# santurini/vsrlab

Measured on AMD Instinct MI355X. Metric: LR frames/sec fwd+bwd, BasicVSR 4x 540p 7-frame clip, 1->8 MI355X, higher is better.
Workload: dtype bf16; 1 GPU; BasicVSR(mid=64,res_blocks=30,x4) fwd+Charbonnier+bwd+clip+Adam, 540x960->2160x3840, 7-frame clip, 2 clips per GPU (BASELINE configs[1]); clips_per_gpu=2, frames=7, res_blocks=30, parallelism=single GPU, arena=full, train_flow=False, trunk_chains=True

## Files before the change

include/vsrlab_hip.h:

```cpp
#ifndef VSRLAB_HIP_H
#define VSRLAB_HIP_H
#include <stddef.h>
#ifdef __cplusplus
extern "C" {
#endif

#define VSR_DT_F32 0
#define VSR_DT_BF16 1

#define VSR_STATUS_OK 0
#define VSR_STATUS_BADARG (-1)
#define VSR_STATUS_UNSUPPORTED (-2)
#define VSR_STATUS_HIP (-3)
#define VSR_STATUS_WORKSPACE (-4)

int vsr_abi_version(void);
const char* vsr_status_string(int status);

typedef struct VsrBasicVSRDesc {
    int n, t, h, w;
    int mid_channels;
    int res_blocks;
    int upscale;
    int dtype;
// ... 66 lines not shown

int vsr_planar_to_pm(int dtype, const float* in, void* out_pm, int N, int Cin, int H, int W, int C,
                     void* stream);
int vsr_pm_to_planar(int dtype, const void* in_pm, float* out, int N, int Cout, int H, int W, int C,
                     void* stream);

int vsr_conv3x3_c64_fwd(int dtype, const void* x_pm, const float* w, const float* b, void* wpack,
                        void* y_pm, const void* res_pm, int act, int N, int H, int W, void* stream);

size_t vsr_conv3x3_c64_chain_sync_bytes(int nlayers, int N, int H, int W);
int vsr_conv3x3_c64_chain_fwd(const void* images, const void* wpack, const float* bias, int nlayers, int N, int H, int W,
                              void* sync, void* stream);
int vsr_conv3x3_c64_dgrad(int dtype, const void* dy_pm, const float* w, void* wpack, void* dx_pm,
                          const void* res_pm, const void* aux_pm, int mask_mode, int N, int H,
                          int W, void* stream);
int vsr_conv_layer_fwd(int dtype, int ks, const void* x_pm, int cin_pm, const float* lr_planar, const float* w,
                       const float* b, int cin_real, int cout_real, void* wpack, void* y_pm, int cd, float* y_planar,
                       int act, float slope, int pixel_shuffle, int N, int H, int W, void* stream);
size_t vsr_conv_layer_bwd_scratch_bytes(int dtype, int N, int H, int W, int pixel_shuffle);
int vsr_conv_layer_bwd(int dtype, int ks, const void* x_pm, int cin_pm, const float* lr_planar, const float* w, int cin_real,
                       int cout_real, const void* y_pm, const float* y_planar, const void* dy_pm, const float* dy_planar, int cd,
                       int act, float slope, int pixel_shuffle, void* dx_pm, float* dlr_planar, float* gw, float* gb,
                       void* scratch, size_t scratch_bytes, int N, int H, int W, void* stream);
size_t vsr_conv3x3_c64_wgrad_slab_floats(void);
int vsr_conv3x3_c64_wgrad(int dtype, const void* x_pm, const void* dy_pm, float* gw, float* gb,
                          float* slab, int N, int H, int W, void* stream);

size_t vsr_charbonnier_scratch_floats(void);
int vsr_charbonnier_fwd_bwd(const float* sr, const float* hr, float* dsr, float* loss, float* scratch, long long numel,
                            float eps, void* stream);
// ... 47 lines not shown
```

vsrlab_amd/_lib.py:

```python
import ctypes
import os
from ctypes import c_char_p, c_float, c_int, c_longlong, c_size_t, c_void_p

_HERE = os.path.dirname(os.path.abspath(__file__))
LIB_PATH = os.environ.get("VSRLAB_AMD_LIB") or os.path.join(_HERE, "lib", "libvsrlab_hip.so")

DT_F32 = 0
DT_BF16 = 1


class BasicVSRDesc(ctypes.Structure):
    _fields_ = [("n", c_int), ("t", c_int), ("h", c_int), ("w", c_int), ("mid_channels", c_int),
                ("res_blocks", c_int), ("upscale", c_int), ("dtype", c_int), ("arena_mode", c_int)]


class DiscDesc(ctypes.Structure):
    _fields_ = [("n", c_int), ("h", c_int), ("w", c_int), ("mid_ch", c_int), ("dtype", c_int)]


class AttnDesc(ctypes.Structure):
    _fields_ = [(k, c_int) for k in ("B", "N", "heads", "head_dim", "q0", "k0", "o0", "Nq", "Nk", "Cout", "c_off", "nW", "Nm")] + \
               [("scale", c_float), ("dtype", c_int), ("mask_packed", c_int), ("mask_value", c_float)]


# ... 19 lines not shown
    "vsr_cleaner_narrow_workspace_bytes": (c_size_t, [c_int, c_int, c_int, c_int, c_int, c_int, c_int, c_int]),
    "vsr_cleaner_forward": (c_int, [c_int, c_int, c_int, c_int, c_int, c_int, c_int, _P, c_int, _P, _P, _P, c_size_t, c_int, _P]),
    "vsr_cleaner_backward": (c_int, [c_int, c_int, c_int, c_int, c_int, c_int, c_int, _P, c_int, _P, _P, _P, _P, c_size_t, _P]),
    "vsr_flow_warp_fwd": (c_int, [c_int, _P, _P, _P, c_int, c_int, c_int, c_int, _P]),
    "vsr_flow_warp_bwd": (c_int, [c_int, _P, _P, _P, c_int, c_int, c_int, c_int, _P]),
    "vsr_flow_warp_bwd_flow": (c_int, [c_int, _P, _P, _P, _P, c_int, c_int, c_int, c_int, _P]),
    "vsr_flow_warp_fwd_ex": (c_int, [c_int, _P, _P, _P, c_int, c_int, c_int, c_int, c_int, _P]),
    "vsr_flow_warp_bwd_ex": (c_int, [c_int, _P, _P, _P, c_int, c_int, c_int, c_int, c_int, _P]),
    "vsr_flow_warp_bwd_flow_ex": (c_int, [c_int, _P, _P, _P, _P, c_int, c_int, c_int, c_int, c_int, _P]),
    "vsr_planar_to_pm": (c_int, [c_int, _P, _P, c_int, c_int, c_int, c_int, c_int, _P]),
    "vsr_pm_to_planar": (c_int, [c_int, _P, _P, c_int, c_int, c_int, c_int, c_int, _P]),
    "vsr_conv3x3_c64_fwd": (c_int, [c_int, _P, _P, _P, _P, _P, _P, c_int, c_int, c_int, c_int, _P]),
    "vsr_conv3x3_c64_chain_sync_bytes": (c_size_t, [c_int, c_int, c_int, c_int]),
    "vsr_conv3x3_c64_chain_fwd": (c_int, [_P, _P, _P, c_int, c_int, c_int, c_int, _P, _P]),
    "vsr_conv3x3_c64_dgrad": (c_int, [c_int, _P, _P, _P, _P, _P, _P, c_int, c_int, c_int, c_int, _P]),
    "vsr_conv_layer_fwd": (c_int, [c_int, c_int, _P, c_int, _P, _P, _P, c_int, c_int, _P, _P, c_int, _P, c_int, c_float, c_int, c_int, c_int, c_int, _P]),
    "vsr_conv_layer_bwd_scratch_bytes": (c_size_t, [c_int, c_int, c_int, c_int, c_int]),
    "vsr_conv_layer_bwd": (c_int, [c_int, c_int, _P, c_int, _P, _P, c_int, c_int, _P, _P, _P, _P, c_int, c_int, c_float, c_int, _P, _P, _P, _P,
                                   _P, c_size_t, c_int, c_int, c_int, _P]),
    "vsr_conv3x3_c64_wgrad_slab_floats": (c_size_t, []),
    "vsr_conv3x3_c64_wgrad": (c_int, [c_int, _P, _P, _P, _P, _P, c_int, c_int, c_int, _P]),
    "vsr_charbonnier_scratch_floats": (c_size_t, []),
    "vsr_charbonnier_fwd_bwd": (c_int, [_P, _P, _P, _P, _P, c_longlong, c_float, _P]),
    "vsr_optim_scratch_floats": (c_size_t, []),
    "vsr_adam_clip_step": (c_int, [_P, _P, _P, _P, c_longlong, c_float, c_float, c_float, c_float, c_float, c_int, c_float,
                                   c_float, _P, _P, _P]),
    "vsr_grad_norm": (c_int, [_P, c_longlong, c_float, _P, _P, _P]),
    "vsr_resize_bilinear": (c_int, [_P, _P, c_longlong, c_int, c_int, c_int, c_int, _P]),
    "vsr_disc_workspace_bytes": (c_size_t, [ctypes.POINTER(DiscDesc), c_int]),
    "vsr_disc_forward": (c_int, [ctypes.POINTER(DiscDesc), _P, c_int, _P, _P, _P, c_size_t, c_int, _P]),
# ... 36 lines not shown
```

vsrlab_amd/csrc/common.h:

```cpp
#pragma once
#include <hip/hip_runtime.h>
#include <stdint.h>

#define VSR_OK 0
#define VSR_ERR_BADARG (-1)
#define VSR_ERR_UNSUPPORTED (-2)
#define VSR_ERR_HIP (-3)
#define VSR_ERR_WORKSPACE (-4)

#define VSR_F32 0
#define VSR_BF16 1

typedef __bf16 bf16_t;
typedef __attribute__((ext_vector_type(8))) __bf16 bf16x8_t;
typedef __attribute__((ext_vector_type(4))) __bf16 bf16x4_t;
typedef __attribute__((ext_vector_type(4))) short s16x4_t;
typedef __attribute__((ext_vector_type(16))) float f32x16_t;
typedef __attribute__((ext_vector_type(4))) float f32x4_t;

#define VSR_MAX_SRC 4
#define VSR_MAX_Z 4

enum { ACT_NONE = 0, ACT_RELU = 1, ACT_LEAKY = 2 };
enum { MASK_NONE = 0, MASK_RELU = 1, MASK_LEAKY = 2, MASK_RELU_BITS = 3, MASK_LEAKY_BITS = 4 };
// ... 18 lines not shown
    int cout_real;
    int act;
    const void* res[VSR_MAX_Z];
    const void* aux[VSR_MAX_Z];
    int mask_mode;
    const float* pres;
    const float* base_lr;
    long long base_nstride;
    int base_h, base_w, base_scale;
    void* sign_out[VSR_MAX_Z];
    const void* sign_bits[VSR_MAX_Z];
    float leaky_slope;
    int planar_c;
    int unshuffle;
    long long unshuffle_plane;
};
static inline __host__ __device__ float vsr_slope(float s) { return s != 0.f ? s : 0.1f; }

#define VSR_WG_MAXSEG 8
struct WgradArgs {
    const void* x[VSR_WG_MAXSEG];
    const void* dy[VSR_WG_MAXSEG];
    long long x_nstride, dy_nstride;
    int nseg;
    int N, H, W;
    int x_step, x_oy, x_ox, Hx, Wx;
    int dy_step, dy_oy, dy_ox, Hy, Wy;
    float* slab;
    int tap_begin;
    int x_ctotal, x_coff;
// ... 83 lines not shown
```

vsrlab_amd/csrc/conv3x3_persist.hip:

```cpp
#include "common.h"
#include <type_traits>

namespace {

constexpr int PTW = 32, PTH = 8, PNT = 512;
constexpr int PTWH = PTW + 2, PTHH = PTH + 2, PNPIX = PTHH * PTWH;
constexpr int W_BYTES = 9 * 64 * 64 * 2;
constexpr int IN_BYTES = PNPIX * 128;
constexpr int BIAS_OFF = W_BYTES + 2 * IN_BYTES;
constexpr int P_LDS = BIAS_OFF + 256;
constexpr int IN_CHUNKS = PNPIX * 8;
constexpr int NPIECE_T = (IN_CHUNKS + 63) / 64;
constexpr int NPIECE_W = (NPIECE_T + 3) / 4;

__device__ uint4 g_conv_zero_chunk[2];

template <int ACT> __device__ __forceinline__ float p_act(float v, float slope) {
    if (ACT == ACT_RELU) return v > 0.f ? v : 0.f;
    if (ACT == ACT_LEAKY) return v > 0.f ? v : slope * v;
    return v;
}

#ifdef VSR_STAMPS
__device__ unsigned long long g_stamps[256 * 8 * 8];
// ... 55 lines not shown
__device__ __forceinline__ unsigned pk_max_i16(unsigned a, unsigned b) { unsigned r; asm("v_pk_max_i16 %0, %1, %2" : "=v"(r) : "v"(a), "v"(b)); return r; }
__device__ __forceinline__ unsigned pk_min_u16(unsigned a, unsigned b) { unsigned r; asm("v_pk_min_u16 %0, %1, %2" : "=v"(r) : "v"(a), "v"(b)); return r; }
__device__ __forceinline__ unsigned pk_mul_lo_u16(unsigned a, unsigned b) { unsigned r; asm("v_pk_mul_lo_u16 %0, %1, %2" : "=v"(r) : "v"(a), "v"(b)); return r; }

#ifdef VSR_ABL
#define P_DMA_AUX (((VSR_ABL >> 8) & 1) ? 2 : 0)
#define P_NT_STORE ((VSR_ABL >> 9) & 1)
#else
#define P_DMA_AUX 0
#define P_NT_STORE 0
#endif
#define GLDS16(src, dst)                                                                              \
    __builtin_amdgcn_global_load_lds((const __attribute__((address_space(1))) void*)(src),            \
                                     (__attribute__((address_space(3))) void*)(dst), 16, 0, P_DMA_AUX)

template <int ACT, bool HAS_RES, int MASK>
__global__ __launch_bounds__(PNT, 1) void conv3x3_c64_persist_kernel(const ConvArgs ka) {
    extern __shared__ __attribute__((aligned(16))) char smem[];

    const int z = blockIdx.y;
    struct {
        int N, H, W, Ws, Wd, in_step, out_step, src_ox0, src_oy0, out_oxz, out_oyz, bias_zstride, unshuffle;
        long long src_nstride0, dst_nstride, w_zstride, plane;
        unsigned long long src0, wpack, resz, auxz, sign_bitsz, dstz, sign_outz, bias; float leaky_slope;
    } a = {ka.N, ka.H, ka.W, ka.Ws, ka.Wd, ka.in_step, ka.out_step, ka.src_ox[0], ka.src_oy[0], ka.out_ox[z], ka.out_oy[z], ka.bias_zstride, ka.unshuffle,
           ka.src_nstride[0], ka.dst_nstride, ka.w_zstride, ka.unshuffle_plane,
           (unsigned long long)ka.src[0], (unsigned long long)ka.wpack, (unsigned long long)ka.res[z], (unsigned long long)ka.aux[z],
           (unsigned long long)ka.sign_bits[z], (unsigned long long)ka.dst[z], (unsigned long long)ka.sign_out[z], (unsigned long long)ka.bias, ka.leaky_slope};
    asm volatile("" : "+s"(a.N), "+s"(a.H), "+s"(a.W), "+s"(a.Ws), "+s"(a.Wd), "+s"(a.in_step), "+s"(a.out_step), "+s"(a.src_ox0), "+s"(a.src_oy0),
                 "+s"(a.out_oxz), "+s"(a.out_oyz), "+s"(a.bias_zstride), "+s"(a.unshuffle), "+s"(a.src_nstride0), "+s"(a.dst_nstride), "+s"(a.w_zstride), "+s"(a.plane));
    asm volatile("" : "+s"(a.src0), "+s"(a.wpack), "+s"(a.resz), "+s"(a.auxz), "+s"(a.sign_bitsz), "+s"(a.dstz), "+s"(a.sign_outz), "+s"(a.bias), "+s"(a.leaky_slope));
#define GP(T, x) ((__attribute__((address_space(1))) T*)(x))
    const int tid = threadIdx.x, lane = tid & 63, wave = tid >> 6;
    const int role = __builtin_amdgcn_readfirstlane(wave >> 2);
    const int w4 = wave & 3;
    const int l15 = lane & 15, q = lane >> 4;
    const int pxl = (l15 >= 4 && l15 < 12) ? 2 * (l15 - 4) : (l15 < 4 ? 2 * l15 + 1 : 2 * (l15 - 8) + 1);
    char* lds_w = smem;
#ifdef VSR_STAMPS
    const unsigned long long st_begin = stamp();
    unsigned long long st_sum[8] = {0, 0, 0, 0, 0, 0, 0, 0};
#endif
    char* lds_t = smem + W_BYTES;
#ifdef VSR_ABL
    unsigned long long clk_t0 = 0, clk_r0 = 0;
// ... 22 lines not shown
        *reinterpret_cast<u32x4_t*>(lds_w + tap * 8192 + (r * 8 + (c ^ ((r >> 1) & 7))) * 16) = wv[i];                     \
    }

    if (role == 1) {
        const auto* src = GP(const char, a.src0);
        const auto* zsrc = GP(const char, g_conv_zero_chunk);
        int rel[NPIECE_W];
#pragma unroll
        for (int i = 0; i < NPIECE_W; ++i) {
            const int idx = (w4 + 4 * i) * 64 + lane;
            const int ty = idx / (8 * PTWH), rem = idx - ty * (8 * PTWH);
            const int c = rem / PTWH, tx = rem - c * PTWH;
            const int dx = (tx - 1) * a.in_step + a.src_ox0;
            rel[i] = (((((ty - 1) * a.in_step + a.src_oy0) * WSs + (dx >> 5)) * 8 + c) * 256 + (dx & 31) * 8) * 2;
        }
        auto issue = [&](const TileIter& it, int buf) {
            const int n = it.n, ty0 = it.ty * PTH, tx0 = it.tx * PTW;
            const auto* org = src + ((long long)n * a.src_nstride0 + pm_off(ty0 * a.in_step, tx0 * a.in_step, 0, a.Ws, 64)) * 2;
            char* dstb = lds_t + buf * IN_BYTES;
            if (ty0 >= 1 && ty0 + PTH < a.H && tx0 >= 1 && tx0 + PTW < a.W) {
#pragma unroll
                for (int i = 0; i < NPIECE_W; ++i) {
                    const int piece = w4 + 4 * i;
                    if (piece < NPIECE_T && piece * 64 + lane < IN_CHUNKS) GLDS16(org + rel[i], dstb + piece * 1024);
                }
            } else {
#pragma unroll
                for (int i = 0; i < NPIECE_W; ++i) {
                    const int piece = w4 + 4 * i;
                    const int idx = piece * 64 + lane;
                    const int ty = idx / (8 * PTWH), rem = idx - ty * (8 * PTWH);
                    const int tx = rem % PTWH;
                    const int vy = ty0 + ty - 1, vx = tx0 + tx - 1;
                    const auto* s = (vy >= 0 && vy < a.H && vx >= 0 && vx < a.W) ? org + rel[i] : zsrc;
                    if (piece < NPIECE_T && idx < IN_CHUNKS) GLDS16(s, dstb + piece * 1024);
                }
            }
        };
        int cur = 0;
        TileIter it;
        it.init(walk.first, walk.stride, ntx, nty);
        STAMP(q0);
        if (it.tile < walk.end) issue(it, 0);
        STAMP(q1);
        STAMP_ADD(1, st_begin, q0);
        asm volatile("s_waitcnt vmcnt(0)" ::: "memory");
        STAMP(q3);
        __syncthreads();
        STAMP_ADD(2, st_begin, q1); STAMP_ADD(4, q1, q3);
        while (it.tile < walk.end) {
            STAMP(t0);
            it.advance(walk.stride, ntx, nty);
            if (it.tile < walk.end && !ABL(3)) issue(it, cur ^ 1);
            STAMP(p1);
            asm volatile("s_waitcnt vmcnt(0)" ::: "memory");
            STAMP(p2);
            __syncthreads();
            STAMP(p3);
            STAMP_ADD(5, t0, p1); STAMP_ADD(6, p1, p2); STAMP_ADD(7, p2, p3);
            cur ^= 1;
        }
    } else {
        STAMP(m0);
        u32x4_t wv[WCH];
        W_LOAD(wv)
        unsigned a_lo[2], a_hi[2];
#pragma unroll
        for (int kk = 0; kk < 2; ++kk) {
            a_lo[kk] = (unsigned)((l15 * 8 + ((4 * kk + q) ^ ((l15 >> 1) & 7))) * 16);
            a_hi[kk] = a_lo[kk] + 6 * 8192;
        }
        const int b_lane = w4 * 2 * (PTWH * 128) + q * (PTWH * 16) + pxl * 16;
        int loff[4];
#pragma unroll
        for (int nb = 0; nb < 4; ++nb) {
            const int dx = ((nb & 1) * 16 + pxl) * a.out_step + a.out_oxz;
            loff[nb] = ((((w4 * 2 + (nb >> 1)) * a.out_step) * WSd + (dx >> 5)) * 8 + q) * 256 + (dx & 31) * 8;
            if (a.unshuffle) {
                const int row = w4 * 2 + (nb >> 1), px = (nb & 1) * 16 + pxl;
                loff[nb] = (int)(((row & 1) * 2 + (px & 1)) * a.plane) + (((row >> 1) * pm_ws(a.Wd >> 1)) * 8 + q) * 256 + (px >> 1) * 8;
            }
        }
        W_STORE(wv)
        STAMP(m1);
        STAMP_ADD(6, m0, m1);
        asm volatile("s_waitcnt vmcnt(0)" ::: "memory");
        __syncthreads();
#ifdef VSR_STAMPS
        st_sum[5] = stamp() - st_begin;
#endif
        auto* const dst_z = GP(bf16_t, a.dstz);
        const auto* const res_z = GP(const bf16_t, a.resz);
        const auto* const aux_z = GP(const bf16_t, a.auxz);
        const auto* const sbits_z = GP(const u32x2_t, a.sign_bitsz);
        auto* const sout_z = GP(u32x2_t, a.sign_outz);
        const float slope = vsr_slope(a.leaky_slope);

        f32x4_t bvec[4];
#pragma unroll
        for (int mb = 0; mb < 4; ++mb) bvec[mb] = *reinterpret_cast<const f32x4_t*>(smem + BIAS_OFF + (mb * 16 + 4 * q) * 4);
        bf16x8_t idA[2];
#pragma unroll
        for (int hb = 0; hb < 2; ++hb)
#pragma unroll
            for (int j = 0; j < 8; ++j) idA[hb][j] = (bf16_t)((q == (l15 >> 2) && j == 4 * hb + (l15 & 3)) ? 1.f : 0.f);
        constexpr bool RES_MFMA = HAS_RES && !ABL(4);

        int cur = 0;
        TileIter it;
        for (it.init(walk.first, walk.stride, ntx, nty); it.tile < walk.end; it.advance(walk.stride, ntx, nty)) {
            STAMP(t0);
            const int tile = it.tile, n = it.n, ty0 = it.ty * PTH, tx0 = it.tx * PTW;
            const long long tbase = a.unshuffle ? (long long)n * a.dst_nstride + pm_off(ty0 >> 1, tx0 >> 1, 0, a.Wd >> 1, 64)
                                                : (long long)n * a.dst_nstride + pm_off(ty0 * a.out_step + a.out_oyz, tx0 * a.out_step, 0, a.Wd, 64);
            const bool full = ty0 + PTH <= a.H && tx0 + PTW <= a.W;
            bool ok[4];
            constexpr bool BITS = MASK == MASK_RELU_BITS || MASK == MASK_LEAKY_BITS;
            constexpr bool LATE_MASK = HAS_RES && MASK != MASK_NONE && !BITS;
            u32x4_t rr[2][4], mm[2][4];
            u32x2_t sbits = {0u, 0u};
            if (BITS) sbits = sbits_z[(long long)tile * 256 + w4 * 64 + lane];
#pragma unroll
            for (int nb = 0; nb < 4; ++nb) ok[nb] = (tx0 + (nb & 1) * 16 + pxl < a.W) && (ty0 + w4 * 2 + (nb >> 1) < a.H);
#define CV_OPERANDS(OKN)                                                                                               \
            _Pragma("unroll") for (int nb = 0; nb < 4; ++nb) {                                                         \
                if (OKN) {                                                                                             \
                    _Pragma("unroll") for (int k = 0; k < 2; ++k) {                                                    \
                        const long long o = tbase + loff[nb] + k * 1024;                                               \
                        if (HAS_RES) rr[k][nb] = *GP(const u32x4_t, res_z + o);                                        \
                        if (MASK != MASK_NONE && !LATE_MASK && !BITS) mm[k][nb] = *GP(const u32x4_t, aux_z + o);       \
                    }                                                                                                  \
                }                                                                                                      \
            }
            if (HAS_RES || (MASK != MASK_NONE && !LATE_MASK && !BITS)) {
                if (full) { CV_OPERANDS(true) } else { CV_OPERANDS(ok[nb]) }
            }
#undef CV_OPERANDS
            STAMP(t1);

            f32x4_t acc[4][4];

            bf16x8_t fa[2][4], fb[2][4];
            const unsigned bb = (unsigned)(W_BYTES + cur * IN_BYTES + b_lane);
#define DSR(dst, addr, imm) asm volatile("ds_read_b128 %0, %1 offset:%2" : "=v"(dst) : "v"(addr), "i"(imm))
#define CV_LOADA(tap_, kk_, slot, mb)                                                                                  \
            if (!(ABL(2) && tap_ >= 6) && !(ABL(6) && tap_ + kk_ > 0)) DSR(fa[slot][mb], (tap_ < 6 ? a_lo[kk_] : a_hi[kk_]), (tap_ < 6 ? tap_ : tap_ - 6) * 8192 + (mb) * 2048);
#define CV_LOADB(ky_, kx_, kk_, slot, nb)                                                                              \
            if (!(ABL(0) && ky_ == 2) && !(ABL(6) && ky_ + kx_ + kk_ > 0)) DSR(fb[slot][nb], bb, (((nb) >> 1) + ky_) * (PTWH * 128) + kk_ * (4 * PTWH * 16) + (((nb) & 1) * 16 + kx_) * 16);
#define CV_LOAD(s, slot)                                                                                               \
// ... 15 lines not shown
            __builtin_amdgcn_sched_barrier(0);
#define CV_STEP(s)                                                                                                     \
            {                                                                                                          \
                if (!ABL(7)) asm volatile("s_waitcnt lgkmcnt(0)" ::: "memory");              \
                __builtin_amdgcn_sched_barrier(0);                                                                     \
                CV_ML_A(s, 0, 0, 0) CV_ML_A(s, 0, 1, 1) CV_ML_A(s, 0, 2, 2) CV_ML_A(s, 0, 3, 3)                        \
                CV_ML_B(s, 1, 0, 0) CV_ML_B(s, 1, 1, 1) CV_ML_B(s, 1, 2, 2) CV_ML_B(s, 1, 3, 3)                        \
                CV_MFMA(s, 2, 0) CV_MFMA(s, 2, 1) CV_MFMA(s, 2, 2) CV_MFMA(s, 2, 3)                                    \
                CV_MFMA(s, 3, 0) CV_MFMA(s, 3, 1) CV_MFMA(s, 3, 2) CV_MFMA(s, 3, 3)                                    \
                __builtin_amdgcn_sched_barrier(0);                                                                     \
            }
            asm volatile("s_waitcnt lgkmcnt(0)" ::: "memory");
            __builtin_amdgcn_sched_barrier(0);
            CV_LOAD(0, 0)
            CV_STEP(0) CV_STEP(1) CV_STEP(2) CV_STEP(3) CV_STEP(4) CV_STEP(5) CV_STEP(6) CV_STEP(7) CV_STEP(8)
            CV_STEP(9) CV_STEP(10) CV_STEP(11) CV_STEP(12) CV_STEP(13) CV_STEP(14) CV_STEP(15) CV_STEP(16) CV_STEP(17)
#undef CV_ML_A
#undef CV_ML_B
#undef CV_STEP
#undef CV_MFMA
#undef CV_LOAD
#undef CV_LOADB
#undef CV_LOADA
#undef DSR
            STAMP(t2);

            if (HAS_RES || MASK != MASK_NONE) __builtin_amdgcn_s_waitcnt(0x0F70);
            if constexpr (RES_MFMA) {
#pragma unroll
                for (int nb = 0; nb < 4; ++nb)
#pragma unroll
                    for (int mb = 0; mb < 4; ++mb)
                        acc[mb][nb] = __builtin_amdgcn_mfma_f32_16x16x32_bf16(idA[mb & 1], __builtin_bit_cast(bf16x8_t, rr[mb >> 1][nb]), acc[mb][nb], 0, 0, 0);
            }
            unsigned sout[2] = {0u, 0u};
            const unsigned k11 = 0x00010001u;
            auto epilogue = [&](auto FULL) {
#pragma unroll
            for (int nb = 0; nb < 4; ++nb) {
                if (decltype(FULL)::value || ok[nb]) {
                    auto* dst = dst_z + tbase + loff[nb];
#pragma unroll
                    for (int k = 0; k < 2; ++k) {
                        float v[8];
#pragma unroll
                        for (int j = 0; j < 4; ++j) { v[j] = acc[2 * k][nb][j]; v[4 + j] = acc[2 * k + 1][nb][j]; }
                        const unsigned wbits = k ? sbits.y : sbits.x;
                        unsigned ow[4];
// ... 16 lines not shown
#pragma unroll
                            for (int jj = 0; jj < 4; ++jj)
                                ow[jj] = pk_mul_lo_u16(pk_bf16(v[2 * jj], v[2 * jj + 1]), (wbits >> (4 * nb + jj)) & k11);
                        } else {
#pragma unroll
                            for (int j = 0; j < 8; ++j) v[j] = p_act<ACT>(v[j], slope);
                            if (HAS_RES && !(RES_MFMA && ACT == ACT_NONE)) {
                                const unsigned rw[4] = {rr[k][nb].x, rr[k][nb].y, rr[k][nb].z, rr[k][nb].w};
#pragma unroll
                                for (int jj = 0; jj < 4; ++jj) { v[2 * jj] += bf_lo(rw[jj]); v[2 * jj + 1] += bf_hi(rw[jj]); }
                            }
                            if (ACT != ACT_NONE && !HAS_RES && !ABL(1)) {
#pragma unroll
                                for (int j = 0; j < 8; ++j) sout[k] |= (v[j] > 0.f ? 1u : 0u) << (4 * nb + (j >> 1) + 16 * (j & 1));
                            }
                            if (BITS) {
                                const float neg = MASK == MASK_LEAKY_BITS ? slope : 0.f;
#pragma unroll
                                for (int j = 0; j < 8; ++j) v[j] *= ((wbits >> (4 * nb + (j >> 1) + 16 * (j & 1))) & 1u) ? 1.f : neg;
                            } else if (MASK != MASK_NONE) {
                                const float neg = MASK == MASK_LEAKY ? slope : 0.f;
                                u32x4_t mq = mm[k][nb];
                                if (LATE_MASK) mq = *GP(const u32x4_t, aux_z + tbase + loff[nb] + k * 1024);
                                const unsigned mw[4] = {mq.x, mq.y, mq.z, mq.w};
#pragma unroll
                                for (int jj = 0; jj < 4; ++jj) {
                                    v[2 * jj] *= (bf_lo(mw[jj]) > 0.f ? 1.f : neg);
                                    v[2 * jj + 1] *= (bf_hi(mw[jj]) > 0.f ? 1.f : neg);
                                }
                            }
#pragma unroll
                            for (int jj = 0; jj < 4; ++jj) ow[jj] = pk_bf16(v[2 * jj], v[2 * jj + 1]);
                        }
                        const u32x4_t o = {ow[0], ow[1], ow[2], ow[3]};
                        if (P_NT_STORE) __builtin_nontemporal_store(o, GP(u32x4_t, dst + k * 1024));
                        else if (!ABL(5)) *GP(u32x4_t, dst + k * 1024) = o;
                        else asm volatile("" :: "v"(o.x), "v"(o.y), "v"(o.z), "v"(o.w));
                    }
                }
            }
            };
            if (full) epilogue(std::true_type{}); else epilogue(std::false_type{});
            if (ACT != ACT_NONE && !HAS_RES && sout_z && !ABL(1)) sout_z[(long long)tile * 256 + w4 * 64 + lane] = u32x2_t{sout[0], sout[1]};
            STAMP(t3);
            __syncthreads();
            cur ^= 1;
            STAMP(t4);
            STAMP_ADD(1, t0, t1); STAMP_ADD(2, t1, t2); STAMP_ADD(3, t2, t3); STAMP_ADD(4, t3, t4);
        }
    }
// ... 27 lines not shown
        const int yy = ty0 + 2 * w4 + (nb >> 1), xx = tx0 + (nb & 1) * 16 + pxl;
        if (yy < H && xx < W) {
#pragma unroll
            for (int k = 0; k < 2; ++k) {
                const uint4 v = *reinterpret_cast<const uint4*>(x + (long long)n * pm_image_elems(H, W, 64) + pm_off(yy, xx, 4 * k + q, W, 64));
                const unsigned vw[4] = {v.x, v.y, v.z, v.w};
#pragma unroll
                for (int jj = 0; jj < 4; ++jj)
                    out[k] |= ((bf_lo(vw[jj]) > 0.f ? 1u : 0u) | (bf_hi(vw[jj]) > 0.f ? 0x10000u : 0u)) << (4 * nb + jj);
            }
        }
    }
    bits[gid] = make_uint2(out[0], out[1]);
}

template <int ACT, bool HAS_RES, int MASK>
static int launch_persist(const ConvArgs& a, int num_cus, hipStream_t st) {
    auto kern = conv3x3_c64_persist_kernel<ACT, HAS_RES, MASK>;
    static VsrDevOnce once;
    { const int rc = vsr_set_max_dynamic_lds(once, reinterpret_cast<const void*>(kern), P_LDS); if (rc != VSR_OK) return rc; }
    const int tiles = a.N * cdiv(a.W, PTW) * cdiv(a.H, PTH);
    int gx = num_cus / a.nz;
    gx &= ~7;
    if (gx < 8) gx = num_cus / a.nz;
    if (gx < 1) gx = 1;
    if (gx > tiles) gx = tiles;
    hipLaunchKernelGGL(kern, dim3(gx, a.nz), dim3(PNT), P_LDS, st, a);
    HIP_CHECK_RET(hipGetLastError());
    return VSR_OK;
}

}

// ... 33 lines not shown
    }
#define PERSIST_CASE(ACT, RES, MASK) if (a.act == ACT && res == RES && mask == MASK) return launch_persist<ACT, RES, MASK>(a, num_cus, st);
    PERSIST_CASE(ACT_RELU, false, MASK_NONE)
    PERSIST_CASE(ACT_NONE, true, MASK_NONE)
    PERSIST_CASE(ACT_LEAKY, false, MASK_NONE)
    PERSIST_CASE(ACT_NONE, false, MASK_NONE)
    PERSIST_CASE(ACT_NONE, false, MASK_RELU)
    PERSIST_CASE(ACT_NONE, false, MASK_RELU_BITS)
    PERSIST_CASE(ACT_NONE, true, MASK_LEAKY)
    PERSIST_CASE(ACT_NONE, true, MASK_LEAKY_BITS)
    PERSIST_CASE(ACT_NONE, false, MASK_LEAKY)
#undef PERSIST_CASE
    return VSR_ERR_UNSUPPORTED;
}

int vsr_launch_sign_bits_c64(const void* x_pm, void* bits, int N, int H, int W, hipStream_t st) {
    if (!x_pm || !bits || N < 1 || H < 1 || W < 1) return VSR_ERR_BADARG;
    const long long total = (long long)N * cdiv(W, PTW) * cdiv(H, PTH) * 256;
    hipLaunchKernelGGL(sign_bits_c64_kernel, dim3((unsigned)((total + 255) / 256)), dim3(256), 0, st, (const bf16_t*)x_pm, (uint2*)bits, N, H, W);
    HIP_CHECK_RET(hipGetLastError());
    return VSR_OK;
}
```

vsrlab_amd/csrc/engine.hip:

```cpp
#include <vector>
#include "kernels.h"
#include "../../include/vsrlab_hip.h"

namespace {

struct Bump {
    size_t off = 0;
    size_t take(size_t bytes) {
        size_t o = off;
        off += (bytes + 255) & ~size_t(255);
        return o;
    }
};

inline size_t esize(int dtype) { return dtype == VSR_BF16 ? 2 : 4; }

constexpr int C = 64;
constexpr int NSPY = 5;
const int SPY_CI[NSPY] = {8, 32, 64, 32, 16}, SPY_CO[NSPY] = {32, 64, 32, 16, 2};
const int SPY_CIP[NSPY] = {16, 32, 64, 32, 16}, SPY_COP[NSPY] = {32, 64, 32, 32, 32};
const int SPY_CD[NSPY] = {32, 64, 32, 16, 0};
const int SPY_DK[NSPY] = {32, 64, 32, 16, 16}, SPY_DROWS[NSPY] = {32, 32, 64, 32, 32};

struct SpyPlan {
// ... 170 lines not shown
                    G1[dir].assign((size_t)t * rb, 0); DX[dir].assign((size_t)t * (rb + 1), 0);
                    for (int i = 0; i < t; ++i) {
                        for (int k = 0; k < rb; ++k) G1[dir][(size_t)i * rb + k] = b.take(a1);
                        for (int k = 1; k <= rb; ++k) DX[dir][(size_t)i * (rb + 1) + k] = b.take(a1);
                    }
                } else {
                    G1[dir] = G1[0]; DX[dir] = DX[0];
                }
            }
            dFeatB.assign(t, 0); dFF.assign(t, 0);
            for (int i = 0; i < t; ++i) { dFeatB[i] = b.take(a1); dFF[i] = b.take(a1); }
            for (int dir = 0; dir < 2; ++dir) { S[dir] = b.take(s_elems * 8); dWp[dir] = b.take(a1); }
            far_cnt = b.take((size_t)2 * 32 * 4);
            G_C0 = b.take(a4h); G_P = b.take(a1);
            unsh = !diet && dtype == VSR_BF16 && !vsr_env().generic_conv && C == 64;
            const size_t gu1 = unsh && 4 * a2 > a4 ? 4 * a2 : a4, gu0 = unsh && 4 * a1 > a2 ? 4 * a1 : a2;
            if (ups == 2) { if (diet) { G_U1 = C0[0]; G_U0 = U1[0]; } else { G_U1 = b.take(gu1); G_U0 = b.take(gu0); } }
            else { G_U0 = diet ? C0[0] : b.take(gu0); G_U1 = G_U0; }
            hrdef = unsh;
            GU1f.assign(t, G_U1); GU0f.assign(t, G_U0); GPf.assign(t, G_P);
            if (hrdef)
                for (int i = 1; i < t; ++i) {
                    GU0f[i] = b.take(gu0);
                    GU1f[i] = ups == 2 ? b.take(gu1) : GU0f[i];
                    GPf[i] = b.take(a1);
                }
            int cp, xp, stride;
            vsr_wgrad_slab_dims(3, 64, 64, &cp, &xp, &stride);
            for (int k = 0; k < 2; ++k) slab[k] = b.take((size_t)VSR_WGRAD_NWG * stride * 4);
        }
// ... 43 lines not shown
        if (unshuffle) set_unshuffle(a, N, H, W);
        if (p.C != 64) return vsr_launch_conv(dtype, 3, 1, p.C, p.C, 0, p.CO, EPI_NHWC, a, st);
        const int rc = vsr_launch_conv(dtype, 3, 1, 64, 64, 0, 64, EPI_NHWC, a, st);
        if (rc == VSR_OK && sign_out && dtype == VSR_BF16 && vsr_env().generic_conv) return vsr_launch_sign_bits_c64(y, sign_out, N, H, W, st);
        return rc;
    }
    int conv_ps(const void* x, size_t wpack, const float* bias4, void* y, int N, int H, int W) const {
        const int C = p.C;
        ConvArgs a = base(N, H, W);
        a.src[0] = x; a.wpack = at(wpack); a.w_zstride = 9 * p.CO * C; a.bias = bias4; a.bias_zstride = C; a.nz = 4;
        a.out_step = 2; a.Hd = 2 * H; a.Wd = 2 * W; a.dst_nstride = pm_image_elems(2 * H, 2 * W, C);
        for (int z = 0; z < 4; ++z) { a.dst[z] = y; a.out_oy[z] = z >> 1; a.out_ox[z] = z & 1; }
        return vsr_launch_conv(dtype, 3, 1, C, C, 0, p.CO, EPI_NHWC, a, st);
    }
    int conv_ps_dgrad(const void* dy, size_t wpackd, void* dx, const void* aux, int mask, int N, int H, int W, const void* sign_bits = nullptr,
                      bool dy_planes = false, bool dx_planes = false) const {
        const int C = p.C;
        if (dtype == VSR_BF16 && C == 64) {
            for (int z = 0; z < 4; ++z) {
                ConvArgs a = base(N, H, W);
                if (dy_planes) {
                    a.src[0] = (const char*)dy + (size_t)z * plane_elems(N, 2 * H, 2 * W) * p.es;
                } else {
                    a.in_step = 2; a.Hs = 2 * H; a.Ws = 2 * W;
                    a.src[0] = dy; a.src_oy[0] = z >> 1; a.src_ox[0] = z & 1; a.src_nstride[0] = pm_image_elems(2 * H, 2 * W, C);
                }
                a.wpack = at(wpackd + (size_t)z * 9 * C * C * p.es); a.dst[0] = dx;
                a.res[0] = z > 0 ? dx : nullptr;
                if (dx_planes) set_unshuffle(a, N, H, W);
                if (z == 3) { a.aux[0] = aux; a.mask_mode = mask; a.sign_bits[0] = aux ? sign_bits : nullptr; }
                int rc = vsr_launch_conv(dtype, 3, 1, 64, 64, 0, 64, EPI_NHWC, a, st);
                if (rc != VSR_OK) return rc;
// ... 1119 lines not shown
    return vsr_launch_conv3x3_chain(a, vsr_num_cus(), (hipStream_t)stream);
}

int vsr_conv3x3_c64_dgrad(int dtype, const void* dy_pm, const float* w, void* wpack, void* dx_pm, const void* res_pm,
                          const void* aux_pm, int mask_mode, int N, int H, int W, void* stream) {
    if (bad_dtype(dtype) || !dy_pm || !w || !wpack || !dx_pm || bad_dims(N, H, W) || mask_mode < MASK_NONE || mask_mode > MASK_LEAKY ||
        (mask_mode != MASK_NONE && !aux_pm))
        return VSR_ERR_BADARG;
    hipStream_t st = (hipStream_t)stream;
    CK(vsr_launch_pack_weights(dtype, w, wpack, 9, C, C, C, C, C, 0, 1, 0, 1, st));
    ConvArgs a = plain64(dy_pm, wpack, nullptr, dx_pm, N, H, W);
    a.res[0] = res_pm; a.aux[0] = aux_pm; a.mask_mode = mask_mode;
    return vsr_launch_conv(dtype, 3, 1, 64, 64, 0, 64, EPI_NHWC, a, st);
}

size_t vsr_conv_layer_bwd_scratch_bytes(int dtype, int N, int H, int W, int pixel_shuffle) {
    if (bad_dtype(dtype) || bad_dims(N, H, W)) return 0;
    const size_t es = esize(dtype);
    const int s = pixel_shuffle ? 2 : 1;
    int cp3, xp3, stride3;
    vsr_wgrad_slab_dims(3, 64, 64, &cp3, &xp3, &stride3);
    return (size_t)49 * 64 * 64 * 4 * es + (size_t)N * pm_image_elems(s * H, s * W, C) * es + (size_t)VSR_WGRAD_NWG * stride3 * 4 + 1024;
}

int vsr_conv_layer_bwd(int dtype, int ks, const void* x_pm, int cin_pm, const float* lr_planar, const float* w, int cin_real, int cout_real,
                       const void* y_pm, const float* y_planar, const void* dy_pm, const float* dy_planar, int cd, int act, float slope,
                       int pixel_shuffle, void* dx_pm, float* dlr_planar, float* gw, float* gb, void* scratch, size_t scratch_bytes,
                       int N, int H, int W, void* stream) {
    if (bad_dtype(dtype) || !w || !scratch || bad_dims(N, H, W) || (!x_pm && !lr_planar) || (!dy_pm && !dy_planar) || act < ACT_NONE || act > ACT_LEAKY)
        return VSR_ERR_BADARG;
// ... 239 lines not shown
```

vsrlab_amd/csrc/kernels.h:

```cpp
#pragma once
#include "common.h"

int vsr_launch_conv(int dtype, int ks, int nsrc, int ca, int cb, int last_planar, int cout_t, int epi,
                    const ConvArgs& a, hipStream_t st);
int vsr_launch_sign_bits_c64(const void* x_pm, void* bits, int N, int H, int W, hipStream_t st);

enum { CHAIN_RELU = 0,
       CHAIN_SKIP = 1,
       CHAIN_MASK = 2 };
#define VSR_CHAIN_MAX_LAYERS 64
struct ChainLayer { unsigned src, dst, res, sbits, sout, w, bias; int variant; };
struct ChainArgs {
    char* base;
    unsigned* sync;
    int N, H, W, nlayers;
    ChainLayer layer[VSR_CHAIN_MAX_LAYERS];
};
size_t vsr_chain_sync_bytes(int nlayers, int N, int H, int W);
int vsr_launch_conv3x3_chain(const ChainArgs& a, int num_cus, hipStream_t st);
void vsr_wgrad_slab_dims(int ks, int cx, int cout, int* coutp, int* cxp, int* stride);
int vsr_launch_wgrad(int dtype, int ks, int cx, int x_planar, int cout, int dy_planar, const WgradArgs& a, int nwg,
                     int* nslabs, hipStream_t st);
int vsr_launch_wgrad_reduce(const float* slab, int nwg, int ks, int cx, int cout, int cout_real, int cin_real, float* gw,
                            int I_total, int i_off, int o_mul, int o_add, float* gb, int accumulate, hipStream_t st);
// ... 68 lines not shown
```

Before: 59.12 LR frames/s.

## Fuse four pixel-shuffle dgrad sub-convolutions into one persistent kernel pass

Adds a PS4 variant of the persistent 3x3 c64 conv kernel. For each tile it loops over the four pixel-shuffle phases, reloading per-phase weights into LDS and keeping the running sum in registers instead of writing and re-reading it as a residual. This replaces four separate dgrad launches, and their intermediate global-memory traffic, with a single launch. The cost is weight reloads per tile, extra barriers and more register pressure. The engine also disables unshuffle when offsets could overflow 32-bit.

```diff
diff --git a/include/vsrlab_hip.h b/include/vsrlab_hip.h
--- a/include/vsrlab_hip.h
+++ b/include/vsrlab_hip.h
@@ -104,6 +104,8 @@
 int vsr_conv3x3_c64_dgrad(int dtype, const void* dy_pm, const float* w, void* wpack, void* dx_pm,
                           const void* res_pm, const void* aux_pm, int mask_mode, int N, int H,
                           int W, void* stream);
+int vsr_conv3x3_c64_ps_dgrad(int fused, const void* dy_pm, int dy_planes, const float* w, void* wpack, void* dx_pm, int dx_planes,
+                             const void* aux_pm, void* bits, int N, int H, int W, void* stream);
 int vsr_conv_layer_fwd(int dtype, int ks, const void* x_pm, int cin_pm, const float* lr_planar, const float* w,
                        const float* b, int cin_real, int cout_real, void* wpack, void* y_pm, int cd, float* y_planar,
                        int act, float slope, int pixel_shuffle, int N, int H, int W, void* stream);
diff --git a/vsrlab_amd/_lib.py b/vsrlab_amd/_lib.py
--- a/vsrlab_amd/_lib.py
+++ b/vsrlab_amd/_lib.py
@@ -57,6 +57,7 @@
     "vsr_conv3x3_c64_chain_sync_bytes": (c_size_t, [c_int, c_int, c_int, c_int]),
     "vsr_conv3x3_c64_chain_fwd": (c_int, [_P, _P, _P, c_int, c_int, c_int, c_int, _P, _P]),
     "vsr_conv3x3_c64_dgrad": (c_int, [c_int, _P, _P, _P, _P, _P, _P, c_int, c_int, c_int, c_int, _P]),
+    "vsr_conv3x3_c64_ps_dgrad": (c_int, [c_int, _P, c_int, _P, _P, _P, c_int, _P, _P, c_int, c_int, c_int, _P]),
     "vsr_conv_layer_fwd": (c_int, [c_int, c_int, _P, c_int, _P, _P, _P, c_int, c_int, _P, _P, c_int, _P, c_int, c_float, c_int, c_int, c_int, c_int, _P]),
     "vsr_conv_layer_bwd_scratch_bytes": (c_size_t, [c_int, c_int, c_int, c_int, c_int]),
     "vsr_conv_layer_bwd": (c_int, [c_int, c_int, _P, c_int, _P, _P, c_int, c_int, _P, _P, _P, _P, c_int, c_int, c_float, c_int, _P, _P, _P, _P,
diff --git a/vsrlab_amd/csrc/common.h b/vsrlab_amd/csrc/common.h
--- a/vsrlab_amd/csrc/common.h
+++ b/vsrlab_amd/csrc/common.h
@@ -56,6 +56,7 @@
     int planar_c;
     int unshuffle;
     long long unshuffle_plane;
+    long long ps_off[4];
 };
 static inline __host__ __device__ float vsr_slope(float s) { return s != 0.f ? s : 0.1f; }
 
diff --git a/vsrlab_amd/csrc/conv3x3_persist.hip b/vsrlab_amd/csrc/conv3x3_persist.hip
--- a/vsrlab_amd/csrc/conv3x3_persist.hip
+++ b/vsrlab_amd/csrc/conv3x3_persist.hip
@@ -93,21 +93,22 @@
     __builtin_amdgcn_global_load_lds((const __attribute__((address_space(1))) void*)(src),            \
                                      (__attribute__((address_space(3))) void*)(dst), 16, 0, P_DMA_AUX)
 
-template <int ACT, bool HAS_RES, int MASK>
+template <int ACT, bool HAS_RES, int MASK, bool PS4 = false>
 __global__ __launch_bounds__(PNT, 1) void conv3x3_c64_persist_kernel(const ConvArgs ka) {
     extern __shared__ __attribute__((aligned(16))) char smem[];
 
     const int z = blockIdx.y;
     struct {
         int N, H, W, Ws, Wd, in_step, out_step, src_ox0, src_oy0, out_oxz, out_oyz, bias_zstride, unshuffle;
-        long long src_nstride0, dst_nstride, w_zstride, plane;
+        long long src_nstride0, dst_nstride, w_zstride, plane, ps_off1, ps_off2, ps_off3;
         unsigned long long src0, wpack, resz, auxz, sign_bitsz, dstz, sign_outz, bias; float leaky_slope;
     } a = {ka.N, ka.H, ka.W, ka.Ws, ka.Wd, ka.in_step, ka.out_step, ka.src_ox[0], ka.src_oy[0], ka.out_ox[z], ka.out_oy[z], ka.bias_zstride, ka.unshuffle,
-           ka.src_nstride[0], ka.dst_nstride, ka.w_zstride, ka.unshuffle_plane,
+           ka.src_nstride[0], ka.dst_nstride, ka.w_zstride, ka.unshuffle_plane, PS4 ? ka.ps_off[1] : 0, PS4 ? ka.ps_off[2] : 0, PS4 ? ka.ps_off[3] : 0,
            (unsigned long long)ka.src[0], (unsigned long long)ka.wpack, (unsigned long long)ka.res[z], (unsigned long long)ka.aux[z],
            (unsigned long long)ka.sign_bits[z], (unsigned long long)ka.dst[z], (unsigned long long)ka.sign_out[z], (unsigned long long)ka.bias, ka.leaky_slope};
     asm volatile("" : "+s"(a.N), "+s"(a.H), "+s"(a.W), "+s"(a.Ws), "+s"(a.Wd), "+s"(a.in_step), "+s"(a.out_step), "+s"(a.src_ox0), "+s"(a.src_oy0),
                  "+s"(a.out_oxz), "+s"(a.out_oyz), "+s"(a.bias_zstride), "+s"(a.unshuffle), "+s"(a.src_nstride0), "+s"(a.dst_nstride), "+s"(a.w_zstride), "+s"(a.plane));
+    if (PS4) asm volatile("" : "+s"(a.ps_off1), "+s"(a.ps_off2), "+s"(a.ps_off3));
     asm volatile("" : "+s"(a.src0), "+s"(a.wpack), "+s"(a.resz), "+s"(a.auxz), "+s"(a.sign_bitsz), "+s"(a.dstz), "+s"(a.sign_outz), "+s"(a.bias), "+s"(a.leaky_slope));
 #define GP(T, x) ((__attribute__((address_space(1))) T*)(x))
     const int tid = threadIdx.x, lane = tid & 63, wave = tid >> 6;
@@ -160,9 +161,10 @@
             const int dx = (tx - 1) * a.in_step + a.src_ox0;
             rel[i] = (((((ty - 1) * a.in_step + a.src_oy0) * WSs + (dx >> 5)) * 8 + c) * 256 + (dx & 31) * 8) * 2;
         }
-        auto issue = [&](const TileIter& it, int buf) {
+        auto issue = [&](const TileIter& it, int buf, int zz = 0) {
             const int n = it.n, ty0 = it.ty * PTH, tx0 = it.tx * PTW;
-            const auto* org = src + ((long long)n * a.src_nstride0 + pm_off(ty0 * a.in_step, tx0 * a.in_step, 0, a.Ws, 64)) * 2;
+            const long long poff = !PS4 || zz == 0 ? 0 : zz == 1 ? a.ps_off1 : zz == 2 ? a.ps_off2 : a.ps_off3;
+            const auto* org = src + ((long long)n * a.src_nstride0 + pm_off(ty0 * a.in_step, tx0 * a.in_step, 0, a.Ws, 64)) * 2 + poff;
             char* dstb = lds_t + buf * IN_BYTES;
             if (ty0 >= 1 && ty0 + PTH < a.H && tx0 >= 1 && tx0 + PTW < a.W) {
 #pragma unroll
@@ -186,6 +188,45 @@
         int cur = 0;
         TileIter it;
         it.init(walk.first, walk.stride, ntx, nty);
+        if constexpr (PS4) {
+            int woff[18];
+#pragma unroll
+            for (int i = 0; i < 18; ++i) {
+                const int piece = i < 10 ? w4 + 4 * i : 40 + w4 + 4 * (i - 10);
+                const int slot = piece * 64 + lane;
+                const int tap = slot >> 9, r = (slot >> 3) & 63, c = (slot & 7) ^ ((r >> 1) & 7);
+                woff[i] = ((tap * 64 + pm_acc_chan(r >> 4, r & 15)) * 8 + c) * 16;
+            }
+            auto issue_w = [&](int zz, int g) {
+                const auto* wb = GP(const char, a.wpack) + (long long)zz * a.w_zstride * 2;
+                if (g == 0) {
+#pragma unroll
+                    for (int i = 0; i < 10; ++i) GLDS16(wb + woff[i], lds_w + (w4 + 4 * i) * 1024);
+                } else {
+#pragma unroll
+                    for (int i = 10; i < 18; ++i) GLDS16(wb + woff[i], lds_w + (40 + w4 + 4 * (i - 10)) * 1024);
+                }
+            };
+            if (it.tile < walk.end) { issue_w(0, 0); issue(it, 0, 0); }
+            asm volatile("s_waitcnt vmcnt(0)" ::: "memory");
+            __syncthreads();
+            int zp = 0;
+            while (it.tile < walk.end) {
+                issue_w(zp, 1);
+                TileIter nx = it;
+                int nzp = zp + 1;
+                if (nzp == 4) { nzp = 0; nx.advance(walk.stride, ntx, nty); }
+                const bool more = nx.tile < walk.end;
+                if (more) issue(nx, cur ^ 1, nzp);
+                if (!more) asm volatile("s_waitcnt vmcnt(0)\n\ts_barrier" ::: "memory");
+                else if (w4 < 3) asm volatile("s_waitcnt vmcnt(11)\n\ts_barrier" ::: "memory");
+                else asm volatile("s_waitcnt vmcnt(10)\n\ts_barrier" ::: "memory");
+                if (more) issue_w(nzp, 0);
+                asm volatile("s_waitcnt vmcnt(0)" ::: "memory");
+                __syncthreads();
+                it = nx; zp = nzp; cur ^= 1;
+            }
+        } else {
         STAMP(q0);
         if (it.tile < walk.end) issue(it, 0);
         STAMP(q1);
@@ -206,10 +247,11 @@
             STAMP_ADD(5, t0, p1); STAMP_ADD(6, p1, p2); STAMP_ADD(7, p2, p3);
             cur ^= 1;
         }
+        }
     } else {
         STAMP(m0);
         u32x4_t wv[WCH];
-        W_LOAD(wv)
+        if constexpr (!PS4) { W_LOAD(wv) }
         unsigned a_lo[2], a_hi[2];
 #pragma unroll
         for (int kk = 0; kk < 2; ++kk) {
@@ -227,7 +269,7 @@
                 loff[nb] = (int)(((row & 1) * 2 + (px & 1)) * a.plane) + (((row >> 1) * pm_ws(a.Wd >> 1)) * 8 + q) * 256 + (px >> 1) * 8;
             }
         }
-        W_STORE(wv)
+        if constexpr (!PS4) { W_STORE(wv) }
         STAMP(m1);
         STAMP_ADD(6, m0, m1);
         asm volatile("s_waitcnt vmcnt(0)" ::: "memory");
@@ -251,10 +293,13 @@
 #pragma unroll
             for (int j = 0; j < 8; ++j) idA[hb][j] = (bf16_t)((q == (l15 >> 2) && j == 4 * hb + (l15 & 3)) ? 1.f : 0.f);
         constexpr bool RES_MFMA = HAS_RES && !ABL(4);
+        u32x4_t run[2][4];
 
         int cur = 0;
         TileIter it;
-        for (it.init(walk.first, walk.stride, ntx, nty); it.tile < walk.end; it.advance(walk.stride, ntx, nty)) {
+        for (it.init(walk.first, walk.stride, ntx, nty); it.tile < walk.end; it.advance(walk.stride, ntx, nty))
+          for (int zp = 0; zp < (PS4 ? 4 : 1); ++zp) {
+            const bool last = !PS4 || zp == 3;
             STAMP(t0);
             const int tile = it.tile, n = it.n, ty0 = it.ty * PTH, tx0 = it.tx * PTW;
             const long long tbase = a.unshuffle ? (long long)n * a.dst_nstride + pm_off(ty0 >> 1, tx0 >> 1, 0, a.Wd >> 1, 64)
@@ -265,7 +310,7 @@
             constexpr bool LATE_MASK = HAS_RES && MASK != MASK_NONE && !BITS;
             u32x4_t rr[2][4], mm[2][4];
             u32x2_t sbits = {0u, 0u};
-            if (BITS) sbits = sbits_z[(long long)tile * 256 + w4 * 64 + lane];
+            if (BITS && last) sbits = sbits_z[(long long)tile * 256 + w4 * 64 + lane];
 #pragma unroll
             for (int nb = 0; nb < 4; ++nb) ok[nb] = (tx0 + (nb & 1) * 16 + pxl < a.W) && (ty0 + w4 * 2 + (nb >> 1) < a.H);
 #define CV_OPERANDS(OKN)                                                                                               \
@@ -273,12 +318,12 @@
                 if (OKN) {                                                                                             \
                     _Pragma("unroll") for (int k = 0; k < 2; ++k) {                                                    \
                         const long long o = tbase + loff[nb] + k * 1024;                                               \
-                        if (HAS_RES) rr[k][nb] = *GP(const u32x4_t, res_z + o);                                        \
+                        if (HAS_RES && !PS4) rr[k][nb] = *GP(const u32x4_t, res_z + o);                                \
                         if (MASK != MASK_NONE && !LATE_MASK && !BITS) mm[k][nb] = *GP(const u32x4_t, aux_z + o);       \
                     }                                                                                                  \
                 }                                                                                                      \
             }
-            if (HAS_RES || (MASK != MASK_NONE && !LATE_MASK && !BITS)) {
+            if ((HAS_RES && !PS4) || (MASK != MASK_NONE && !LATE_MASK && !BITS)) {
                 if (full) { CV_OPERANDS(true) } else { CV_OPERANDS(ok[nb]) }
             }
 #undef CV_OPERANDS
@@ -324,6 +369,7 @@
             __builtin_amdgcn_sched_barrier(0);
             CV_LOAD(0, 0)
             CV_STEP(0) CV_STEP(1) CV_STEP(2) CV_STEP(3) CV_STEP(4) CV_STEP(5) CV_STEP(6) CV_STEP(7) CV_STEP(8)
+            if (PS4) { asm volatile("s_waitcnt lgkmcnt(0)\n\ts_barrier" ::: "memory"); __builtin_amdgcn_sched_barrier(0); }
             CV_STEP(9) CV_STEP(10) CV_STEP(11) CV_STEP(12) CV_STEP(13) CV_STEP(14) CV_STEP(15) CV_STEP(16) CV_STEP(17)
 #undef CV_ML_A
 #undef CV_ML_B
@@ -335,13 +381,16 @@
 #undef DSR
             STAMP(t2);
 
-            if (HAS_RES || MASK != MASK_NONE) __builtin_amdgcn_s_waitcnt(0x0F70);
+            if (PS4 ? (BITS && last) : (HAS_RES || MASK != MASK_NONE)) __builtin_amdgcn_s_waitcnt(0x0F70);
             if constexpr (RES_MFMA) {
+                if (!PS4 || zp > 0) {
 #pragma unroll
                 for (int nb = 0; nb < 4; ++nb)
 #pragma unroll
                     for (int mb = 0; mb < 4; ++mb)
-                        acc[mb][nb] = __builtin_amdgcn_mfma_f32_16x16x32_bf16(idA[mb & 1], __builtin_bit_cast(bf16x8_t, rr[mb >> 1][nb]), acc[mb][nb], 0, 0, 0);
+                        acc[mb][nb] = __builtin_amdgcn_mfma_f32_16x16x32_bf16(idA[mb & 1], __builtin_bit_cast(bf16x8_t, PS4 ? run[mb >> 1][nb] : rr[mb >> 1][nb]),
+                                                                              acc[mb][nb], 0, 0, 0);
+                }
             }
             unsigned sout[2] = {0u, 0u};
             const unsigned k11 = 0x00010001u;
@@ -388,11 +437,11 @@
 #pragma unroll
                                 for (int j = 0; j < 8; ++j) sout[k] |= (v[j] > 0.f ? 1u : 0u) << (4 * nb + (j >> 1) + 16 * (j & 1));
                             }
-                            if (BITS) {
+                            if (BITS && last) {
                                 const float neg = MASK == MASK_LEAKY_BITS ? slope : 0.f;
 #pragma unroll
                                 for (int j = 0; j < 8; ++j) v[j] *= ((wbits >> (4 * nb + (j >> 1) + 16 * (j & 1))) & 1u) ? 1.f : neg;
-                            } else if (MASK != MASK_NONE) {
+                            } else if (MASK != MASK_NONE && last) {
                                 const float neg = MASK == MASK_LEAKY ? slope : 0.f;
                                 u32x4_t mq = mm[k][nb];
                                 if (LATE_MASK) mq = *GP(const u32x4_t, aux_z + tbase + loff[nb] + k * 1024);
@@ -407,7 +456,8 @@
                             for (int jj = 0; jj < 4; ++jj) ow[jj] = pk_bf16(v[2 * jj], v[2 * jj + 1]);
                         }
                         const u32x4_t o = {ow[0], ow[1], ow[2], ow[3]};
-                        if (P_NT_STORE) __builtin_nontemporal_store(o, GP(u32x4_t, dst + k * 1024));
+                        if (PS4 && !last) run[k][nb] = o;
+                        else if (P_NT_STORE) __builtin_nontemporal_store(o, GP(u32x4_t, dst + k * 1024));
                         else if (!ABL(5)) *GP(u32x4_t, dst + k * 1024) = o;
                         else asm volatile("" :: "v"(o.x), "v"(o.y), "v"(o.z), "v"(o.w));
                     }
@@ -465,9 +515,9 @@
     bits[gid] = make_uint2(out[0], out[1]);
 }
 
-template <int ACT, bool HAS_RES, int MASK>
+template <int ACT, bool HAS_RES, int MASK, bool PS4 = false>
 static int launch_persist(const ConvArgs& a, int num_cus, hipStream_t st) {
-    auto kern = conv3x3_c64_persist_kernel<ACT, HAS_RES, MASK>;
+    auto kern = conv3x3_c64_persist_kernel<ACT, HAS_RES, MASK, PS4>;
     static VsrDevOnce once;
     { const int rc = vsr_set_max_dynamic_lds(once, reinterpret_cast<const void*>(kern), P_LDS); if (rc != VSR_OK) return rc; }
     const int tiles = a.N * cdiv(a.W, PTW) * cdiv(a.H, PTH);
@@ -531,6 +581,27 @@
     return VSR_ERR_UNSUPPORTED;
 }
 
+int vsr_launch_conv3x3_c64_ps4_dgrad(ConvArgs a, int num_cus, hipStream_t st) {
+    if (a.N <= 0 || a.H <= 0 || a.W <= 0 || a.nz != 1 || !a.src[0] || !a.dst[0] || !a.wpack || a.bias || a.res[0] || a.act != ACT_NONE) return VSR_ERR_BADARG;
+    if (!(a.in_step == 1 && a.Hs == a.H && a.Ws == a.W) && !(a.in_step == 2 && a.Hs == 2 * a.H && a.Ws == 2 * a.W)) return VSR_ERR_UNSUPPORTED;
+    if (a.src_oy[0] || a.src_ox[0]) return VSR_ERR_UNSUPPORTED;
+    for (int z = 0; z < 4; ++z) {
+        if (!a.src[z] || a.src_nstride[z] != a.src_nstride[0] || (unsigned)a.src_oy[z] >= (unsigned)a.in_step || (unsigned)a.src_ox[z] >= (unsigned)a.in_step)
+            return VSR_ERR_UNSUPPORTED;
+        a.ps_off[z] = ((const char*)a.src[z] - (const char*)a.src[0]) + ((long long)a.src_oy[z] * pm_ws(a.Ws) * 2048 + a.src_ox[z] * 8) * 2;
+    }
+    if (pm_image_elems((PTHH + 2) * a.in_step, a.Ws, 64) * 2 > 0x7fffffffLL || pm_image_elems(2 * PTH + 2, a.Wd, 64) > 0x7fffffffLL)
+        return VSR_ERR_UNSUPPORTED;
+    if (a.out_step != 1 || a.out_ox[0] || a.out_oy[0] || a.Hd != a.H || a.Wd != a.W) return VSR_ERR_UNSUPPORTED;
+    if (a.unshuffle && (a.aux[0] || (a.Hd & 1) || (a.Wd & 1) || a.unshuffle_plane < (long long)a.N * pm_image_elems(a.Hd / 2, a.Wd / 2, 64) ||
+                        a.dst_nstride != pm_image_elems(a.Hd / 2, a.Wd / 2, 64) || 3 * a.unshuffle_plane + pm_image_elems(PTH + 2, a.Wd / 2, 64) > 0x7fffffffLL))
+        return VSR_ERR_UNSUPPORTED;
+    if (!a.aux[0]) return launch_persist<ACT_NONE, true, MASK_NONE, true>(a, num_cus, st);
+    if (a.mask_mode != MASK_LEAKY) return VSR_ERR_UNSUPPORTED;
+    if (a.sign_bits[0]) return launch_persist<ACT_NONE, true, MASK_LEAKY_BITS, true>(a, num_cus, st);
+    return launch_persist<ACT_NONE, true, MASK_LEAKY, true>(a, num_cus, st);
+}
+
 int vsr_launch_sign_bits_c64(const void* x_pm, void* bits, int N, int H, int W, hipStream_t st) {
     if (!x_pm || !bits || N < 1 || H < 1 || W < 1) return VSR_ERR_BADARG;
     const long long total = (long long)N * cdiv(W, PTW) * cdiv(H, PTH) * 256;
diff --git a/vsrlab_amd/csrc/engine.hip b/vsrlab_amd/csrc/engine.hip
--- a/vsrlab_amd/csrc/engine.hip
+++ b/vsrlab_amd/csrc/engine.hip
@@ -208,6 +208,8 @@
             far_cnt = b.take((size_t)2 * 32 * 4);
             G_C0 = b.take(a4h); G_P = b.take(a1);
             unsh = !diet && dtype == VSR_BF16 && !vsr_env().generic_conv && C == 64;
+            if (unsh && 3 * (long long)n * pm_image_elems(scale * h / 2, scale * w / 2, 64) + pm_image_elems(10, scale * w / 2, 64) > 0x7fffffffLL)
+                unsh = false;
             const size_t gu1 = unsh && 4 * a2 > a4 ? 4 * a2 : a4, gu0 = unsh && 4 * a1 > a2 ? 4 * a1 : a2;
             if (ups == 2) { if (diet) { G_U1 = C0[0]; G_U0 = U1[0]; } else { G_U1 = b.take(gu1); G_U0 = b.take(gu0); } }
             else { G_U0 = diet ? C0[0] : b.take(gu0); G_U1 = G_U0; }
@@ -281,8 +283,24 @@
         return vsr_launch_conv(dtype, 3, 1, C, C, 0, p.CO, EPI_NHWC, a, st);
     }
     int conv_ps_dgrad(const void* dy, size_t wpackd, void* dx, const void* aux, int mask, int N, int H, int W, const void* sign_bits = nullptr,
-                      bool dy_planes = false, bool dx_planes = false) const {
+                      bool dy_planes = false, bool dx_planes = false, bool fused = true) const {
         const int C = p.C;
+        if (dtype == VSR_BF16 && C == 64 && fused && !vsr_env().generic_conv) {
+            ConvArgs a = base(N, H, W);
+            for (int z = 0; z < 4; ++z) {
+                if (dy_planes) {
+                    a.src[z] = (const char*)dy + (size_t)z * plane_elems(N, 2 * H, 2 * W) * p.es;
+                } else {
+                    a.in_step = 2; a.Hs = 2 * H; a.Ws = 2 * W;
+                    a.src[z] = dy; a.src_oy[z] = z >> 1; a.src_ox[z] = z & 1; a.src_nstride[z] = pm_image_elems(2 * H, 2 * W, C);
+                }
+            }
+            a.wpack = at(wpackd); a.w_zstride = 9 * C * C; a.dst[0] = dx;
+            if (dx_planes) set_unshuffle(a, N, H, W);
+            a.aux[0] = aux; a.mask_mode = mask; a.sign_bits[0] = aux ? sign_bits : nullptr;
+            const int rc = vsr_launch_conv3x3_c64_ps4_dgrad(a, vsr_num_cus(), st);
+            if (rc != VSR_ERR_UNSUPPORTED) return rc;
+        }
         if (dtype == VSR_BF16 && C == 64) {
             for (int z = 0; z < 4; ++z) {
                 ConvArgs a = base(N, H, W);
@@ -1432,6 +1450,18 @@
     return vsr_launch_conv(dtype, 3, 1, 64, 64, 0, 64, EPI_NHWC, a, st);
 }
 
+int vsr_conv3x3_c64_ps_dgrad(int fused, const void* dy_pm, int dy_planes, const float* w, void* wpack, void* dx_pm, int dx_planes,
+                             const void* aux_pm, void* bits, int N, int H, int W, void* stream) {
+    if (!dy_pm || !w || !wpack || !dx_pm || bad_dims(N, H, W) || (bits && !aux_pm) || (dx_planes && ((H & 1) || (W & 1) || aux_pm)))
+        return VSR_ERR_BADARG;
+    hipStream_t st = (hipStream_t)stream;
+    Plan dummy; dummy.es = esize(VSR_BF16); dummy.C = 64; dummy.CO = 64;
+    const Ctx c{dummy, (char*)wpack, st, VSR_BF16};
+    for (int z = 0; z < 4; ++z) CK(c.pack(w, (size_t)z * 9 * 64 * 64 * 2, 9, 64, 64, 64, 64, 64, 0, 4, z, 1));
+    if (bits) CK(vsr_launch_sign_bits_c64(aux_pm, bits, N, H, W, st));
+    return c.conv_ps_dgrad(dy_pm, 0, dx_pm, aux_pm, MASK_LEAKY, N, H, W, bits, dy_planes != 0, dx_planes != 0, fused != 0);
+}
+
 size_t vsr_conv_layer_bwd_scratch_bytes(int dtype, int N, int H, int W, int pixel_shuffle) {
     if (bad_dtype(dtype) || bad_dims(N, H, W)) return 0;
     const size_t es = esize(dtype);
diff --git a/vsrlab_amd/csrc/kernels.h b/vsrlab_amd/csrc/kernels.h
--- a/vsrlab_amd/csrc/kernels.h
+++ b/vsrlab_amd/csrc/kernels.h
@@ -4,6 +4,7 @@
 int vsr_launch_conv(int dtype, int ks, int nsrc, int ca, int cb, int last_planar, int cout_t, int epi,
                     const ConvArgs& a, hipStream_t st);
 int vsr_launch_sign_bits_c64(const void* x_pm, void* bits, int N, int H, int W, hipStream_t st);
+int vsr_launch_conv3x3_c64_ps4_dgrad(ConvArgs a, int num_cus, hipStream_t st);
 
 enum { CHAIN_RELU = 0,
        CHAIN_SKIP = 1,
```

Result: no change. 59.60 LR frames/s, median of 6 (+0.8%).
